# helenypzhang/Subspace-Multimodal-Learning

Measured on AMD Instinct MI355X. Metric: bags/sec fwd+bwd, DeformCrossTransMIL N=10k x 512, higher is better.
Workload: dtype f32

## Files before the change

### include/smml.h

```cpp
#ifndef SMML_H_
#define SMML_H_

#include <stddef.h>

#define SMML_ABI_VERSION 2

#ifdef __cplusplus
extern "C" {
#endif

const char* smml_last_error(void);
int smml_abi_version(void);
int smml_device_check(int device);
void* smml_event_create(void);
int smml_event_destroy(void* ev);
int smml_event_record(void* ev, void* stream);
int smml_event_elapsed_ms(void* start, void* stop, float* ms);

int smml_gemm_f32(const float* A, const float* B, float* C, const float* bias, const float* residual,
                  int M, int N, int K, long long sam, long long sak, long long sbk, long long sbn,
                  long long ldc, long long ldr, int nb0, int nb1, long long sa0, long long sa1,
                  long long sb0, long long sb1, long long sc0, long long sc1, long long sbias0,
                  long long sbias1, int bias_mode, int rows_per_bias, long long bias_ld, int act,
                  int splitk, int accumulate, float alpha, float beta, void* stream);
size_t smml_gemm_f32_det_workspace_bytes(int M, int N, int nb0, int nb1, int splitk);
int smml_gemm_f32_det(const float* A, const float* B, float* C, const float* bias, const float* residual,
                      int M, int N, int K, long long sam, long long sak, long long sbk, long long sbn,
                      long long ldc, long long ldr, int nb0, int nb1, long long sa0, long long sa1,
                      long long sb0, long long sb1, long long sc0, long long sc1, long long sbias0,
                      long long sbias1, int bias_mode, int rows_per_bias, long long bias_ld, int act,
                      int splitk, int accumulate, float alpha, float beta, void* workspace, size_t workspace_bytes,
                      void* stream);
void smml_gemm_force_generic(int on);
void smml_gemm_set_mode(int mode);
int smml_gemm_get_mode(void);
void smml_gemm_set_small_tile(int v);

int smml_gemm_b16(const void* A, const void* B, void* C, const float* bias, int M, int N, int K, long long lda, long long ldb,
                  long long ldc, int trans, int out_bf16, int splitk, void* stream);
void smml_gemm_b16_set_tile(int mode);
void smml_gemm_b16_set_slice_major(int on);
int smml_gemm_b16_batched(const void* A, const void* B, void* C, const float* bias, int M, int N, int K, long long lda, long long ldb,
                          long long ldc, int trans, int out_bf16, int splitk, int nb, long long sa, long long sb, long long sc, void* stream);

int smml_grouped_pointwise_applies(int groups, int cin_g, int cout_g);
int smml_grouped_pointwise_fwd_f32(const float* x, const float* w, float* y, long long rows, int groups, int cin_g, int cout_g, void* stream);
int smml_grouped_pointwise_dx_f32(const float* dy, const float* w, float* dx, long long rows, int groups, int cin_g, int cout_g, void* stream);
size_t smml_grouped_pointwise_dw_workspace_bytes(long long rows, int groups, int cin_g, int cout_g);
int smml_grouped_pointwise_dw_f32(const float* dy, const float* x, float* dw, long long rows, int groups, int cin_g, int cout_g,
                                  void* workspace, size_t workspace_bytes, void* stream);

int smml_layernorm_fwd_f32(const float* x, const float* gamma, const float* beta, float* y, float* mean,
                           float* rstd, long long R, int C, float eps, void* stream);
int smml_layernorm_fwd_mean_f32(const float* x, const float* gamma, const float* beta, float* mean, float* rstd, float* out, int nb,
                                long long n, int C, float eps, void* stream);
size_t smml_layernorm_fwd_mean_det_workspace_bytes(int nb, long long n, int C);
int smml_layernorm_fwd_mean_det_f32(const float* x, const float* gamma, const float* beta, float* mean, float* rstd, float* out, int nb,
                                    long long n, int C, float eps, void* workspace, size_t workspace_bytes, void* stream);
int smml_layernorm_bwd_f32(const float* x, const float* dy, const float* gamma, const float* mean,
                           const float* rstd, float* dx, float* dgamma, float* dbeta, long long R, int C,
                           long long rows_per_dy, float dy_scale, int accumulate_dx, void* stream);
size_t smml_layernorm_bwd_det_workspace_bytes(long long R, int C);
int smml_layernorm_bwd_det_f32(const float* x, const float* dy, const float* gamma, const float* mean,
                               const float* rstd, float* dx, float* dgamma, float* dbeta, long long R, int C,
                               long long rows_per_dy, float dy_scale, int accumulate_dx, void* workspace,
                               size_t workspace_bytes, void* stream);

int smml_colsum_f32(const float* x, float* out, int nb, long long R, int C, float scale, void* stream);
size_t smml_colsum_det_workspace_bytes(int nb, long long R, int C);
int smml_colsum_det_f32(const float* x, float* out, int nb, long long R, int C, float scale, void* workspace,
                        size_t workspace_bytes, void* stream);

int smml_orth_loss_f32(const float* P, const float* Ph, const float* G, const float* Gh, const float* dloss, float* loss,
                       float* dP, float* dPh, float* dG, float* dGh, int B, int D, float gamma, void* stream);

int smml_batchloss_tail_f32(const float* go, const float* gv, const float* dloss, float* loss, float* dgo, float* dgv, int R, int nv,
                            float n_total, void* stream);

int smml_relu_bwd_f32(const float* dy, const float* y, float* dx, long long n, void* stream);

int smml_offsets_out_len(int s, int ks, int r);
int smml_offsets_fwd_f32(const float* q, const float* w0, const float* b0, const float* w2, float* vgrid,
                         float* vs, int B, int Hh, int Ww, int G, int dg, int ks, int r, int posdim,
                         float offset_scale, void* stream);
size_t smml_offsets_bwd_workspace_bytes(int B, int Hh, int Ww, int G, int dg, int ks, int r, int posdim);
int smml_offsets_bwd_f32(const float* q, const float* w0, const float* b0, const float* w2,
                         const float* dvgrid, const float* dvs, float* dq, float* dw0, float* db0,
                         float* dw2, void* workspace, size_t workspace_bytes, int B, int Hh, int Ww, int G, int dg,
                         int ks, int r, int posdim, float offset_scale, int accumulate_dq, void* stream);

int smml_bilinear_sample_fwd_f32(const float* x, const float* vs, float* kv, int B, int Hh, int Ww, int G,
                                 int cg, int J, int posdim, void* stream);
int smml_bilinear_sample_bwd_f32(const float* x, const float* vs, const float* dkv, float* dx, float* dvs,
                                 int B, int Hh, int Ww, int G, int cg, int J, int posdim, void* stream);
size_t smml_bilinear_sample_bwd_det_workspace_bytes(int B, int Hh, int Ww, int G, int J);
int smml_bilinear_sample_bwd_det_f32(const float* x, const float* vs, const float* dkv, float* dx, float* dvs,
                                     void* workspace, size_t workspace_bytes, int B, int Hh, int Ww, int G, int cg,
                                     int J, int posdim, void* stream);
int smml_bilinear_corners_f32(const float* vs, int* cx, int* cy, unsigned char* cm, int n, int Hh, int Ww,
                              int posdim, void* stream);

typedef struct SmmlDeformOpts {
  const unsigned long long* seed_offset;
  int raw_distance;
  const unsigned short* mask_table;
  float mask_table_pmax;
  unsigned short* export_masks;
  int region_lds_cap;
} SmmlDeformOpts;

int smml_deform_attn_nst(int N);
int smml_deform_attn_fwd_f32(const float* q, const float* k, const float* v, const float* vs, const float* gq,
                             const float* w1, const float* b1, const float* w2, const float* b2,
                             const float* w3, const float* b3, float* out, float* lse, float* logits_t,
                             unsigned short* relu_masks, int B, int N, int J, int H, int G, int posdim, float scale,
                             float dropout_p, unsigned long long dropout_seed, void* ev_start, void* ev_stop, void* stream, const SmmlDeformOpts* opts);
size_t smml_deform_attn_bwd_workspace_bytes(int B, int N, int J, int H);
int smml_deform_attn_bwd_f32(const float* q, const float* k, const float* v, const float* vs, const float* gq,
                             const float* w1, const float* b1, const float* w2, const float* b2,
// ... 242 lines not shown
```

### subspace-multimodal-learning_amd/_capi.py

```python
from __future__ import annotations

import ctypes as C
import os
import re
from typing import Optional

import torch

_PKG = os.path.dirname(os.path.abspath(__file__))
LIB_PATH = os.environ.get("SMML_LIB") or os.path.join(_PKG, "lib", "libsmml_hip.so")

HEADER_PATH = os.path.join(os.path.dirname(_PKG), "include", "smml.h")


class DeformOpts(C.Structure):
    """SmmlDeformOpts of include/smml.h: optional behaviour of ONE fused deformable-attention launch, passed with the call.
    _fields_ are the header's, set below."""


_SCALARS = {"int": C.c_int, "long long": C.c_longlong, "unsigned long long": C.c_ulonglong, "float": C.c_float, "size_t": C.c_size_t}


def _ctype(ctext: str, where: str, ret: bool = False):
    t = " ".join(ctext.replace("*", " * ").split())
    if t == "void" and ret:
        return None
    if t == "const char *" and ret:
        return C.c_char_p
    if t == "const SmmlDeformOpts *":
        return C.POINTER(DeformOpts)
    if re.fullmatch(r"(const )?\w+( \w+)* \*", t):
        return C.c_void_p
    if t not in _SCALARS:
        raise RuntimeError(f"include/smml.h: type `{ctext.strip()}` of `{where}` is not one the ctypes binding knows")
    return _SCALARS[t]


def _declarator(text: str, where: str):
    m = re.fullmatch(r"\s*([\w\s]*[\w*])\s*\b([A-Za-z_]\w*)\s*", text)
    if not m or m.group(2) in ("int", "long", "float", "void", "unsigned", "size_t", "char", "short", "const"):
        raise RuntimeError(f"include/smml.h: cannot read `{text.strip()}` of `{where}` as `type name`")
    return m.group(2), _ctype(m.group(1), where), re.sub(r"\bconst\b|\s", "", m.group(1)) == "float*"


def parse_prototypes(text: str, params: Optional[dict] = None) -> dict:
    text = re.sub(r"/\*.*?\*/|//[^\n]*", " ", text, flags=re.S)
    text = re.sub(r"^[ \t]*#.*$", " ", text, flags=re.M)
    text = re.sub(r'extern\s+"C"\s*\{(.*)\}', r"\1", text, flags=re.S)
    sigs = {}
    *protos, tail = text.split(";")
    if tail.strip():
        raise RuntimeError(f"include/smml.h: `{' '.join(tail.split())}` does not end in `;`")
    for proto in protos:
        m = re.fullmatch(r"\s*([\w\s*]+?)\b(smml_\w+)\s*\(([^()]*)\)\s*", proto)
        if not m or m.group(2) in sigs:
            raise RuntimeError(f"include/smml.h: cannot read `{' '.join(proto.split())}` as one prototype `ret smml_name(type name, ...)`")
        ret, name, plist = m.groups()
        decl = [] if plist.strip() == "void" else [_declarator(p, name) for p in plist.split(",")]
        sigs[name] = (_ctype(ret, name, ret=True), [t for _, t, _ in decl])
        if params is not None:
            params[name] = decl
    return sigs


def parse_header(text: str, params: Optional[dict] = None):
    text = re.sub(r"/\*.*?\*/|//[^\n]*", " ", text, flags=re.S)
    abi = re.search(r"^[ \t]*#[ \t]*define[ \t]+SMML_ABI_VERSION[ \t]+(\d+)[ \t]*$", text, re.M)
    struct = re.search(r"typedef\s+struct\s+SmmlDeformOpts\s*\{(.*?)\}\s*SmmlDeformOpts\s*;", text, re.S)
    if not abi or not struct:
        raise RuntimeError("include/smml.h: SMML_ABI_VERSION or struct SmmlDeformOpts not found")
    fields = [_declarator(f, "SmmlDeformOpts")[:2] for f in struct.group(1).split(";") if f.strip()]
    return int(abi.group(1)), fields, parse_prototypes(text[:struct.start()] + text[struct.end():], params)


if not os.path.exists(HEADER_PATH):
    raise RuntimeError(f"{HEADER_PATH} is missing: the ctypes binding is derived from it (it ships with the repository, next to the package)")
PARAMS: dict = {}
with open(HEADER_PATH) as _h:
    ABI_VERSION, DeformOpts._fields_, SIGNATURES = parse_header(_h.read(), PARAMS)

_lib: Optional[C.CDLL] = None


def lib() -> C.CDLL:
    global _lib
    if _lib is None:
        if not os.path.exists(LIB_PATH):
            raise RuntimeError(
                f"{LIB_PATH} is missing: build it with `python -c 'import __graft_entry__ as g; g.build()'` "
                "(hipcc --offload-arch=gfx950); there is no CPU or eager fallback for this path")
        handle = C.CDLL(LIB_PATH)
        for name, (res, args) in SIGNATURES.items():
            fn = getattr(handle, name)
            fn.restype = res
            fn.argtypes = args
        if handle.smml_abi_version() != ABI_VERSION:
            raise RuntimeError(f"{LIB_PATH} implements C-ABI version {handle.smml_abi_version()}, this package binds version {ABI_VERSION}: rebuild it")
        if os.environ.get("SMML_GEMM_MODE"):
            handle.smml_gemm_set_mode(int(os.environ["SMML_GEMM_MODE"]))
        if os.environ.get("SMML_GEMM_SMALL_TILE"):
            handle.smml_gemm_set_small_tile(int(os.environ["SMML_GEMM_SMALL_TILE"]))
        _lib = handle
    return _lib


def deform_opts(seed_offset: Optional[torch.Tensor] = None, log_distance: bool = True, mask_table: Optional[torch.Tensor] = None,
                mask_table_pmax: float = 0.0, export_masks: Optional[torch.Tensor] = None, region_lds_cap: int = 0):
    if seed_offset is None and log_distance and mask_table is None and export_masks is None and not region_lds_cap:
        return None
    if seed_offset is not None and (seed_offset.dtype != torch.int64 or seed_offset.numel() != 1):
        raise RuntimeError("dropout_seed_offset must be a device int64 tensor with one element")
    o = DeformOpts(ptr(seed_offset), 0 if log_distance else 1, ptr(mask_table), float(mask_table_pmax), ptr(export_masks), int(region_lds_cap))
    return C.byref(o)


def check(rc: int, what: str = "") -> None:
    if rc != 0:
        msg = lib().smml_last_error().decode("utf-8", "replace")
        raise RuntimeError(f"smml call failed ({rc}){': ' + what if what else ''}: {msg}")


def ptr(t: Optional[torch.Tensor]):
    if t is None:
        return None
    if not t.is_cuda:
        raise RuntimeError("smml kernels need tensors resident in GPU HBM (got a CPU tensor); "
                           "this path has no CPU fallback")
    if not t.is_contiguous():
        raise RuntimeError("smml kernels need contiguous tensors")
    if t.device.index != torch.cuda.current_device():
        raise RuntimeError(f"smml kernels launch on the current device (cuda:{torch.cuda.current_device()}) but got a tensor on "
                           f"{t.device}; call torch.cuda.set_device first (one process per GPU)")
    return C.c_void_p(t.data_ptr())


def fptr(t: Optional[torch.Tensor]):
    if t is not None and t.dtype != torch.float32:
        raise RuntimeError(f"smml fp32 kernel got dtype {t.dtype}")
    return ptr(t)


def stream(device=None):
    return C.c_void_p(torch.cuda.current_stream(device).cuda_stream)


def _plan(decl):
    return [(pname, fptr if is_float else ptr if ctype is C.c_void_p else None) for pname, ctype, is_float in decl]


_PLANS = {name: _plan(decl) for name, decl in PARAMS.items()}


def bind(name: str, values, params: Optional[dict] = None) -> list:
    out = []
    for pname, conv in _PLANS[name] if params is None else _plan(params[name]):
        try:
            v = values[pname]
        except KeyError:
            raise RuntimeError(f"{name}: no value for its parameter `{pname}`") from None
        out.append(conv(v) if conv is not None and isinstance(v, torch.Tensor) else v)
    return out


def call(name: str, values, keys=None):
    if keys is not None and values.keys() != keys:
        raise RuntimeError(f"{name}: the namespace holds {sorted(values)}, its key set names {sorted(keys)}")
    return getattr(lib(), name)(*bind(name, values))
```

### subspace-multimodal-learning_amd/csrc/gemm.hip

```cpp
#include "smml_common.h"
#include <atomic>

namespace {

constexpr int BM = 128, BN = 64, BK = 16;
constexpr int LDA = BM + 4, LDB = BN + 4;

struct GemmArgs {
  const float* A; const float* B; float* C; const float* bias; const float* residual;
  int M, N, K;
  long long sam, sak, sbk, sbn, ldc, ldr;
  int nb0, nb1;
  long long sa0, sa1, sb0, sb1, sc0, sc1, sbias0, sbias1;
  int bias_mode, rows_per_bias; long long bias_ld;
  int act, splitk; float alpha, beta;
  int atomic;
  int swap_xy;
  long long scs;
};

template <bool GATE>
__device__ __forceinline__ float apply_act(float v, int act, int n, int N) {
  if (act == 1) return fmaxf(v, 0.f);
  if (act == 2) return tanhf(v);
  if constexpr (GATE) {
    if (act == 3 || (act == 4 && 2 * n >= N)) return 1.f / (1.f + expf(-v));
    if (act == 4) return tanhf(v);
  }
  return v;
}

template <bool GATE>
__global__ __launch_bounds__(256) void gemm_f32_kernel(GemmArgs g) {
  __shared__ float As[BK][LDA];
  __shared__ float Bs[BK][LDB];
  const int tid = threadIdx.x, wave = tid >> 6, lane = tid & 63, c = lane & 31, hf = lane >> 5;
  const int zb = blockIdx.z / g.splitk, ks = blockIdx.z - zb * g.splitk;
  const int b0 = zb / g.nb1, b1 = zb - b0 * g.nb1;
  const float* A = g.A + b0 * g.sa0 + b1 * g.sa1;
  const float* B = g.B + b0 * g.sb0 + b1 * g.sb1;
  float* C = g.C + b0 * g.sc0 + b1 * g.sc1 + ks * g.scs;
  const int m0 = (g.swap_xy ? blockIdx.y : blockIdx.x) * BM, n0 = (g.swap_xy ? blockIdx.x : blockIdx.y) * BN;
  const int ktiles = (g.K + BK - 1) / BK;
  const int tps = (ktiles + g.splitk - 1) / g.splitk;
  const int kt0 = ks * tps, kt1 = min(ktiles, kt0 + tps);

  floatx16 acc0 = {0}, acc1 = {0};
  const bool a_kcontig = (g.sak == 1);
  const bool b_kcontig = (g.sbk == 1) && (g.sbn != 1);

  for (int kt = kt0; kt < kt1; ++kt) {
    const int k0 = kt * BK;
    __syncthreads();
    if (a_kcontig) {
      const int k = tid & 15;
#pragma unroll
      for (int i = 0; i < 8; ++i) {
        const int m = (tid >> 4) + 16 * i;
        const int gm = m0 + m, gk = k0 + k;
        As[k][m] = (gm < g.M && gk < g.K) ? A[gm * g.sam + gk] : 0.f;
      }
    } else {
      const int m = tid & 127;
#pragma unroll
      for (int i = 0; i < 8; ++i) {
        const int k = (tid >> 7) + 2 * i;
        const int gm = m0 + m, gk = k0 + k;
        As[k][m] = (gm < g.M && gk < g.K) ? A[gm * g.sam + gk * g.sak] : 0.f;
      }
    }
    if (b_kcontig) {
      const int k = tid & 15;
#pragma unroll
      for (int i = 0; i < 4; ++i) {
        const int n = (tid >> 4) + 16 * i;
        const int gn = n0 + n, gk = k0 + k;
        Bs[k][n] = (gn < g.N && gk < g.K) ? B[gk + gn * g.sbn] : 0.f;
      }
    } else {
      const int n = tid & 63;
#pragma unroll
      for (int i = 0; i < 4; ++i) {
        const int k = (tid >> 6) + 4 * i;
        const int gn = n0 + n, gk = k0 + k;
        Bs[k][n] = (gn < g.N && gk < g.K) ? B[gk * g.sbk + gn * g.sbn] : 0.f;
      }
    }
    __syncthreads();
#pragma unroll
    for (int st = 0; st < BK / 2; ++st) {
      const float a = As[2 * st + hf][wave * 32 + c];
      acc0 = mfma32(a, Bs[2 * st + hf][c], acc0);
      acc1 = mfma32(a, Bs[2 * st + hf][32 + c], acc1);
    }
  }

  const float* bias = g.bias ? g.bias + b0 * g.sbias0 + b1 * g.sbias1 : nullptr;
  const float* res = g.residual ? g.residual + b0 * g.sc0 + b1 * g.sc1 : nullptr;
#pragma unroll
  for (int t = 0; t < 2; ++t) {
    const int n = n0 + 32 * t + c;
// ... 122 lines not shown
    store_tile();
    __syncthreads();
    if (kt + 1 < kt1) load_tile(kt + 1);
    float af[MI][8], bf[NI][8];
#pragma unroll
    for (int mi = 0; mi < MI; ++mi) {
      const int row = wm * (FBM / 2) + mi * 32 + c;
      if (A_KC) {
        const float4 x = *reinterpret_cast<const float4*>(&As[row * A_LD + 8 * hf]);
        const float4 y = *reinterpret_cast<const float4*>(&As[row * A_LD + 8 * hf + 4]);
        af[mi][0] = x.x; af[mi][1] = x.y; af[mi][2] = x.z; af[mi][3] = x.w;
        af[mi][4] = y.x; af[mi][5] = y.y; af[mi][6] = y.z; af[mi][7] = y.w;
      } else {
#pragma unroll
        for (int st = 0; st < 8; ++st) af[mi][st] = As[(8 * hf + st) * A_LD + row];
      }
    }
#pragma unroll
    for (int ni = 0; ni < NI; ++ni) {
      const int col = wn * (BN_ / 2) + ni * 32 + c;
      if (B_KC) {
        const float4 x = *reinterpret_cast<const float4*>(&Bs[col * B_LD + 8 * hf]);
        const float4 y = *reinterpret_cast<const float4*>(&Bs[col * B_LD + 8 * hf + 4]);
        bf[ni][0] = x.x; bf[ni][1] = x.y; bf[ni][2] = x.z; bf[ni][3] = x.w;
        bf[ni][4] = y.x; bf[ni][5] = y.y; bf[ni][6] = y.z; bf[ni][7] = y.w;
      } else {
#pragma unroll
        for (int st = 0; st < 8; ++st) bf[ni][st] = Bs[(8 * hf + st) * B_LD + col];
      }
    }
#pragma unroll
    for (int st = 0; st < 8; ++st)
#pragma unroll
      for (int mi = 0; mi < MI; ++mi)
#pragma unroll
        for (int ni = 0; ni < NI; ++ni) acc[mi][ni] = mfma32(af[mi][st], bf[ni][st], acc[mi][ni]);
  }

  const float* bias = g.bias ? g.bias + b0 * g.sbias0 + b1 * g.sbias1 : nullptr;
  const float* res = g.residual ? g.residual + b0 * g.sc0 + b1 * g.sc1 : nullptr;
  if (!g.atomic && m0 + FBM <= g.M && n0 + BN_ <= g.N) {
#pragma unroll
    for (int mi = 0; mi < MI; ++mi)
#pragma unroll
      for (int ni = 0; ni < NI; ++ni) {
        const int n = n0 + wn * (BN_ / 2) + ni * 32 + c;
        const int mb = m0 + wm * (FBM / 2) + mi * 32;
        float rv[16];
#pragma unroll
        for (int r = 0; r < 16; ++r) rv[r] = res ? res[(long long)(mb + acc_row(r, hf)) * g.ldr + n] : 0.f;
#pragma unroll
        for (int r = 0; r < 16; ++r) {
          const int m = mb + acc_row(r, hf);
          float v = g.alpha * acc[mi][ni][r];
          if (bias) v += (g.bias_mode == 2) ? bias[(m / g.rows_per_bias) * g.bias_ld + n] : bias[n];
          v = apply_act<GATE>(v, g.act, n, g.N);
          C[(long long)m * g.ldc + n] = fmaf(g.beta, rv[r], v);
        }
      }
    return;
  }
#pragma unroll
  for (int mi = 0; mi < MI; ++mi)
#pragma unroll
    for (int ni = 0; ni < NI; ++ni) {
      const int n = n0 + wn * (BN_ / 2) + ni * 32 + c;
      if (n >= g.N) continue;
#pragma unroll
      for (int r = 0; r < 16; ++r) {
        const int m = m0 + wm * (FBM / 2) + mi * 32 + acc_row(r, hf);
        if (m >= g.M) continue;
        float v = g.alpha * acc[mi][ni][r];
        if (g.atomic) {
          if (bias && ks == 0) v += (g.bias_mode == 2) ? bias[(m / g.rows_per_bias) * g.bias_ld + n] : bias[n];
          atomicAdd(&C[m * g.ldc + n], v);
        } else {
          if (bias) v += (g.bias_mode == 2) ? bias[(m / g.rows_per_bias) * g.bias_ld + n] : bias[n];
          v = apply_act<GATE>(v, g.act, n, g.N);
          if (res) v = fmaf(g.beta, res[m * g.ldr + n], v);
          C[m * g.ldc + n] = v;
        }
      }
    }
}

__device__ __forceinline__ uint2v f16_pack4(const float4 v) {
  typedef _Float16 h2 __attribute__((ext_vector_type(2)));
  const float2v a = {v.x, v.y}, b = {v.z, v.w};
  return (uint2v){__builtin_bit_cast(unsigned, __builtin_convertvector(a, h2)), __builtin_bit_cast(unsigned, __builtin_convertvector(b, h2))};
}
__device__ __forceinline__ floatx16 mfma16h(bf16x8 a, bf16x8 b, floatx16 c) {
  typedef _Float16 h8 __attribute__((ext_vector_type(8)));
  return __builtin_amdgcn_mfma_f32_32x32x16_f16(__builtin_bit_cast(h8, a), __builtin_bit_cast(h8, b), c, 0, 0, 0);
}

template <int BN_, bool A_KC, bool B_KC, int TERMS = 3, int FBM = 128, bool F16 = false>
__global__ __launch_bounds__(256, 2) void gemm_bf3_kernel(GemmArgs g) {
  static_assert(!F16 || TERMS == 1, "the fp16 form is single-term");
  constexpr int FBK = 32, NI = BN_ / 64, MI = FBM / 64;
  constexpr int A_LD = A_KC ? (FBK + 8) : (FBM + 32);
  constexpr int B_LD = B_KC ? (FBK + 8) : (BN_ + 32);
  constexpr int A_PLANE = (A_KC ? FBM : FBK) * A_LD, B_PLANE = (B_KC ? BN_ : FBK) * B_LD;
  constexpr int NA = FBM / 32, NB = BN_ / 32, MQ = FBM / 4;
  __shared__ __attribute__((aligned(16))) __bf16 As[TERMS * A_PLANE];
  __shared__ __attribute__((aligned(16))) __bf16 Bs[TERMS * B_PLANE];
  const int tid = threadIdx.x, wave = tid >> 6, lane = tid & 63, c = lane & 31, hf = lane >> 5;
  const int wm = wave >> 1, wn = wave & 1;
  const int zb = blockIdx.z / g.splitk, ks = blockIdx.z - zb * g.splitk;
  const int b0 = zb / g.nb1, b1 = zb - b0 * g.nb1;
  const float* A = g.A + b0 * g.sa0 + b1 * g.sa1;
  const float* B = g.B + b0 * g.sb0 + b1 * g.sb1;
  float* C = g.C + b0 * g.sc0 + b1 * g.sc1 + ks * g.scs;
  const int m0 = (g.swap_xy ? blockIdx.y : blockIdx.x) * FBM, n0 = (g.swap_xy ? blockIdx.x : blockIdx.y) * BN_;
  const int ktiles = (g.K + FBK - 1) / FBK;
  const int tps = (ktiles + g.splitk - 1) / g.splitk;
  const int kt0 = ks * tps, kt1 = min(ktiles, kt0 + tps);

  float4 ra[NA], rb[NB];
  auto load_tile = [&](int kt) {
    const int k0 = kt * FBK;
#pragma unroll
    for (int i = 0; i < NA; ++i) {
      const int idx = tid + 256 * i;
      if (A_KC) {
        const int row = idx >> 3, kq = idx & 7;
        const long long gm = min(m0 + row, g.M - 1);
        ra[i] = (k0 + 4 * kq < g.K) ? *reinterpret_cast<const float4*>(A + gm * g.sam + k0 + 4 * kq) : make_float4(0.f, 0.f, 0.f, 0.f);
      } else {
        const int k = idx / MQ, mq = idx - k * MQ;
        const int gm = m0 + 4 * mq;
        const float* p = A + (long long)min(k0 + k, g.K - 1) * g.sak;
        if (k0 + k >= g.K) ra[i] = make_float4(0.f, 0.f, 0.f, 0.f);
        else if (gm >= g.M) ra[i] = make_float4(0.f, 0.f, 0.f, 0.f);
        else if (gm + 3 < g.M) ra[i] = *reinterpret_cast<const float4*>(p + gm);
        else ra[i] = make_float4(p[min(gm, g.M - 1)], p[min(gm + 1, g.M - 1)], p[min(gm + 2, g.M - 1)], p[min(gm + 3, g.M - 1)]);
      }
    }
#pragma unroll
    for (int i = 0; i < NB; ++i) {
      const int idx = tid + 256 * i;
      if (B_KC) {
        const int row = idx >> 3, kq = idx & 7;
        const long long gn = min(n0 + row, g.N - 1);
        rb[i] = (k0 + 4 * kq < g.K) ? *reinterpret_cast<const float4*>(B + gn * g.sbn + k0 + 4 * kq) : make_float4(0.f, 0.f, 0.f, 0.f);
      } else {
        constexpr int NQ = BN_ / 4;
        const int k = idx / NQ, nq = idx - k * NQ;
        const int gn = n0 + 4 * nq;
        const float* p = B + (long long)min(k0 + k, g.K - 1) * g.sbk;
        if (k0 + k >= g.K) rb[i] = make_float4(0.f, 0.f, 0.f, 0.f);
        else if (gn >= g.N) rb[i] = make_float4(0.f, 0.f, 0.f, 0.f);
        else if (gn + 3 < g.N) rb[i] = *reinterpret_cast<const float4*>(p + gn);
        else rb[i] = make_float4(p[min(gn, g.N - 1)], p[min(gn + 1, g.N - 1)], p[min(gn + 2, g.N - 1)], p[min(gn + 3, g.N - 1)]);
      }
    }
  };
  auto store_tile = [&]() {
#pragma unroll
    for (int i = 0; i < NA; ++i) {
      const int idx = tid + 256 * i;
      const int off = A_KC ? ((idx >> 3) * A_LD + 4 * (idx & 7)) : ((idx / MQ) * A_LD + 4 * (idx % MQ));
      uint2v h, m, l;
      if (F16) h = f16_pack4(ra[i]); else split4_bf3(ra[i], h, m, l);
      *reinterpret_cast<uint2v*>(&As[off]) = h;
      if (TERMS == 3) {
        *reinterpret_cast<uint2v*>(&As[A_PLANE + off]) = m;
// ... 74 lines not shown
        }
    }
  }

  const float* bias = g.bias ? g.bias + b0 * g.sbias0 + b1 * g.sbias1 : nullptr;
  const float* res = g.residual ? g.residual + b0 * g.sc0 + b1 * g.sc1 : nullptr;
  if (!g.atomic && m0 + FBM <= g.M && n0 + BN_ <= g.N) {
#pragma unroll
    for (int mi = 0; mi < MI; ++mi)
#pragma unroll
      for (int ni = 0; ni < NI; ++ni) {
        const int n = n0 + wn * (BN_ / 2) + ni * 32 + c;
        const int mb = m0 + wm * (FBM / 2) + mi * 32;
        float rv[16];
#pragma unroll
        for (int r = 0; r < 16; ++r) rv[r] = res ? res[(long long)(mb + acc_row(r, hf)) * g.ldr + n] : 0.f;
#pragma unroll
        for (int r = 0; r < 16; ++r) {
          const int m = mb + acc_row(r, hf);
          float v = g.alpha * acc[mi][ni][r];
          if (bias) v += (g.bias_mode == 2) ? bias[(m / g.rows_per_bias) * g.bias_ld + n] : bias[n];
          v = apply_act<false>(v, g.act, n, g.N);
          C[(long long)m * g.ldc + n] = fmaf(g.beta, rv[r], v);
        }
      }
    return;
  }
#pragma unroll
  for (int mi = 0; mi < MI; ++mi)
#pragma unroll
    for (int ni = 0; ni < NI; ++ni) {
      const int n = n0 + wn * (BN_ / 2) + ni * 32 + c;
      if (n >= g.N) continue;
#pragma unroll
      for (int r = 0; r < 16; ++r) {
        const int m = m0 + wm * (FBM / 2) + mi * 32 + acc_row(r, hf);
        if (m >= g.M) continue;
        float v = g.alpha * acc[mi][ni][r];
        if (g.atomic) {
          if (bias && ks == 0) v += (g.bias_mode == 2) ? bias[(m / g.rows_per_bias) * g.bias_ld + n] : bias[n];
          atomicAdd(&C[m * g.ldc + n], v);
        } else {
          if (bias) v += (g.bias_mode == 2) ? bias[(m / g.rows_per_bias) * g.bias_ld + n] : bias[n];
          v = apply_act<false>(v, g.act, n, g.N);
          if (res) v = fmaf(g.beta, res[m * g.ldr + n], v);
          C[m * g.ldc + n] = v;
        }
      }
    }
}

__global__ __launch_bounds__(256) void gemm_det_reduce_kernel(const float* __restrict__ part, float* __restrict__ C, int M, int N,
                                                              long long ldc, int nb0, int nb1, long long sc0, long long sc1, int splitk,
                                                              int fold0, int fold1, int accumulate) {
  const int e1 = fold1 ? 1 : nb1;
  const long long mn = (long long)M * N;
  const long long total = (long long)(fold0 ? 1 : nb0) * e1 * mn;
  const long long idx = (long long)blockIdx.x * blockDim.x + threadIdx.x;
  if (idx >= total) return;
  const long long o = idx / mn, r = idx - o * mn;
  const int o0 = (int)(o / e1), o1 = (int)(o - (long long)o0 * e1);
  const int b0a = fold0 ? 0 : o0, b0b = fold0 ? nb0 : o0 + 1;
  const int b1a = fold1 ? 0 : o1, b1b = fold1 ? nb1 : o1 + 1;
  float s = 0.f;
  for (int b0 = b0a; b0 < b0b; ++b0)
    for (int b1 = b1a; b1 < b1b; ++b1) {
      const float* p = part + ((long long)b0 * nb1 + b1) * splitk * mn + r;
      for (int ks = 0; ks < splitk; ++ks) s += p[ks * mn];
    }
  const long long m = r / N, n = r - m * N;
  float* c = C + o0 * sc0 + o1 * sc1 + m * ldc + n;
  *c = accumulate ? *c + s : s;
}

}

static std::atomic<int> g_force_generic{0};
static std::atomic<int> g_mode{0};
extern "C" void smml_gemm_force_generic(int on) { g_force_generic = on; }
extern "C" void smml_gemm_set_mode(int mode) { g_mode = mode; }
extern "C" int smml_gemm_get_mode(void) { return g_mode; }
static std::atomic<int> g_small_tile{0};
extern "C" void smml_gemm_set_small_tile(int v) { g_small_tile = v; }

static int gemm_f32_run(const char* fn, const float* A, const float* B, float* C, const float* bias, const float* residual,
                        int M, int N, int K, long long sam, long long sak, long long sbk, long long sbn,
                        long long ldc, long long ldr, int nb0, int nb1, long long sa0, long long sa1,
                        long long sb0, long long sb1, long long sc0, long long sc1, long long sbias0,
                        long long sbias1, int bias_mode, int rows_per_bias, long long bias_ld, int act,
                        int splitk, int atomic, long long scs, float alpha, float beta, void* stream) {
  SMML_REQUIRE(A && B && C, "%s: null operand", fn);
  SMML_REQUIRE(M > 0 && N > 0 && K > 0 && nb0 > 0 && nb1 > 0, "%s: non-positive size (M=%d N=%d K=%d)", fn, M, N, K);
  SMML_REQUIRE(splitk >= 1, "%s: splitk must be >= 1", fn);
  SMML_REQUIRE(!((atomic || scs) && (act != 0 || residual)), "%s: split-K / accumulate excludes activation/residual", fn);
  SMML_REQUIRE(bias_mode >= 0 && bias_mode <= 2, "%s: bad bias_mode %d", fn, bias_mode);
  SMML_REQUIRE(bias_mode != 2 || rows_per_bias > 0, "%s: rows_per_bias must be positive", fn);
  SMML_REQUIRE(act >= 0 && act <= 4, "%s: bad activation %d", fn, act);
  SMML_REQUIRE(act != 4 || N % 2 == 0, "%s: activation 4 (tanh | sigmoid halves) needs an even N, got %d", fn, N);
  const long long gz = (long long)nb0 * nb1 * splitk;
  const long long gy = (N + BN - 1) / BN, gx = (M + BM - 1) / BM;
  const int swap_xy = gy > 65535;
  SMML_REQUIRE(gz <= 65535 && (swap_xy ? gx : gy) <= 65535,
               "smml_gemm_f32: grid too large (batch*splitk=%lld, row tiles=%lld, col tiles=%lld)", gz, gx, gy);
  GemmArgs g{A, B, C, bias_mode ? bias : nullptr, residual, M, N, K, sam, sak, sbk, sbn, ldc, ldr, nb0, nb1,
             sa0, sa1, sb0, sb1, sc0, sc1, sbias0, sbias1, bias_mode, rows_per_bias > 0 ? rows_per_bias : 1,
             bias_ld, act, splitk, alpha, beta, atomic, swap_xy, scs};
  SMML_REQUIRE(!bias_mode || bias, "smml_gemm_f32: bias_mode set but bias is null");
  auto al4 = [](long long v) { return (v & 3) == 0; };
  auto al16 = [](const void* p) { return (((size_t)p) & 15) == 0; };
  const bool a_kc = (sak == 1), a_mc = (sam == 1 && sak != 1);
  const bool b_kc = (sbk == 1 && sbn != 1), b_nc = (sbn == 1);
  const bool a_ok = al16(A) && al4(sa0) && al4(sa1) && ((a_kc && al4(sam)) || (a_mc && al4(sak)));
  const bool b_ok = al16(B) && al4(sb0) && al4(sb1) && ((b_kc && al4(sbn)) || (b_nc && al4(sbk)));
  const bool k_ok = (!a_kc && !b_kc) || (K % 4) == 0;
  const bool gate = act >= 3;
  if (a_ok && b_ok && k_ok && !g_force_generic) {
    const int bn = (N > 64 && gx * ((N + 127) / 128) * gz >= 1024) ? 128 : 64;
    const long long fy = (N + bn - 1) / bn;
    const bool small = bn == 64 && M > 64 && (g_small_tile == 2 || (g_small_tile == 0 && gx * fy * gz < 512));
    const long long fx = small ? (M + 63) / 64 : gx;
    const int fswap = fy > 65535;
    SMML_REQUIRE((fswap ? fx : fy) <= 65535, "smml_gemm_f32: grid too large");
    g.swap_xy = fswap;
    dim3 grid((unsigned)(fswap ? fy : fx), (unsigned)(fswap ? fx : fy), (unsigned)gz);
    hipStream_t st = (hipStream_t)stream;
    const bool bf3_mode = (g_mode == 2) || (g_mode == 0 && K >= 2048 && M >= 1024 && N >= 1024);
    const bool bf3 = !gate && bf3_mode;
    const bool bf1 = !gate && (g_mode == 3), f1 = !gate && (g_mode == 4);
#define SMML_FAST(BNV, AK, BK2)                                                                   \
  do {                                                                                            \
    if (f1) hipLaunchKernelGGL((gemm_bf3_kernel<BNV, AK, BK2, 1, 128, true>), grid, dim3(256), 0, st, g); \
    else if (bf1) hipLaunchKernelGGL((gemm_bf3_kernel<BNV, AK, BK2, 1>), grid, dim3(256), 0, st, g);   \
    else if (bf3) hipLaunchKernelGGL((gemm_bf3_kernel<BNV, AK, BK2>), grid, dim3(256), 0, st, g); \
    else if (gate) hipLaunchKernelGGL((gemm_f32_fast_kernel<BNV, AK, BK2, 128, true>), grid, dim3(256), 0, st, g); \
    else hipLaunchKernelGGL((gemm_f32_fast_kernel<BNV, AK, BK2>), grid, dim3(256), 0, st, g);     \
  } while (0)
#define SMML_SMALL(AK, BK2)                                                                          \
  do {                                                                                               \
    if (f1) hipLaunchKernelGGL((gemm_bf3_kernel<64, AK, BK2, 1, 64, true>), grid, dim3(256), 0, st, g);   \
    else if (bf1) hipLaunchKernelGGL((gemm_bf3_kernel<64, AK, BK2, 1, 64>), grid, dim3(256), 0, st, g);   \
    else if (bf3) hipLaunchKernelGGL((gemm_bf3_kernel<64, AK, BK2, 3, 64>), grid, dim3(256), 0, st, g); \
    else if (gate) hipLaunchKernelGGL((gemm_f32_fast_kernel<64, AK, BK2, 64, true>), grid, dim3(256), 0, st, g); \
    else hipLaunchKernelGGL((gemm_f32_fast_kernel<64, AK, BK2, 64>), grid, dim3(256), 0, st, g);     \
  } while (0)
    if (small) {
      if (a_kc && b_kc) SMML_SMALL(true, true); else if (a_kc) SMML_SMALL(true, false);
      else if (b_kc) SMML_SMALL(false, true); else SMML_SMALL(false, false);
    } else if (bn == 128) {
      if (a_kc && b_kc) SMML_FAST(128, true, true); else if (a_kc) SMML_FAST(128, true, false);
      else if (b_kc) SMML_FAST(128, false, true); else SMML_FAST(128, false, false);
    } else {
      if (a_kc && b_kc) SMML_FAST(64, true, true); else if (a_kc) SMML_FAST(64, true, false);
      else if (b_kc) SMML_FAST(64, false, true); else SMML_FAST(64, false, false);
    }
#undef SMML_FAST
#undef SMML_SMALL
    SMML_LAUNCH_CHECK("smml_gemm_f32/fast");
    return SMML_OK;
  }
  dim3 grid((unsigned)(swap_xy ? gy : gx), (unsigned)(swap_xy ? gx : gy), (unsigned)gz);
  if (gate) hipLaunchKernelGGL(gemm_f32_kernel<true>, grid, dim3(256), 0, (hipStream_t)stream, g);
  else hipLaunchKernelGGL(gemm_f32_kernel<false>, grid, dim3(256), 0, (hipStream_t)stream, g);
  SMML_LAUNCH_CHECK("smml_gemm_f32");
  return SMML_OK;
}

extern "C" int smml_gemm_f32(const float* A, const float* B, float* C, const float* bias, const float* residual,
                             int M, int N, int K, long long sam, long long sak, long long sbk, long long sbn,
                             long long ldc, long long ldr, int nb0, int nb1, long long sa0, long long sa1,
                             long long sb0, long long sb1, long long sc0, long long sc1, long long sbias0,
                             long long sbias1, int bias_mode, int rows_per_bias, long long bias_ld, int act,
                             int splitk, int accumulate, float alpha, float beta, void* stream) {
  const int atomic = (splitk > 1 || accumulate) ? 1 : 0;
  return gemm_f32_run("smml_gemm_f32", A, B, C, bias, residual, M, N, K, sam, sak, sbk, sbn, ldc, ldr, nb0, nb1, sa0, sa1, sb0, sb1,
                      sc0, sc1, sbias0, sbias1, bias_mode, rows_per_bias, bias_ld, act, splitk, atomic, 0, alpha, beta, stream);
}

extern "C" size_t smml_gemm_f32_det_workspace_bytes(int M, int N, int nb0, int nb1, int splitk) {
  if (M <= 0 || N <= 0 || nb0 <= 0 || nb1 <= 0 || splitk <= 0) return 0;
  return (size_t)nb0 * (size_t)nb1 * (size_t)splitk * (size_t)M * (size_t)N * sizeof(float);
}

extern "C" int smml_gemm_f32_det(const float* A, const float* B, float* C, const float* bias, const float* residual,
                                 int M, int N, int K, long long sam, long long sak, long long sbk, long long sbn,
                                 long long ldc, long long ldr, int nb0, int nb1, long long sa0, long long sa1,
                                 long long sb0, long long sb1, long long sc0, long long sc1, long long sbias0,
                                 long long sbias1, int bias_mode, int rows_per_bias, long long bias_ld, int act,
                                 int splitk, int accumulate, float alpha, float beta, void* workspace, size_t workspace_bytes,
                                 void* stream) {
  SMML_REQUIRE(A && B && C && workspace, "smml_gemm_f32_det: null operand or workspace");
  SMML_REQUIRE(M > 0 && N > 0 && K > 0 && nb0 > 0 && nb1 > 0 && splitk >= 1, "smml_gemm_f32_det: non-positive size (M=%d N=%d K=%d)", M, N, K);
  SMML_REQUIRE(!bias && !residual && bias_mode == 0 && act == 0, "smml_gemm_f32_det: the reduced product takes no bias, activation or residual");
  SMML_REQUIRE((long long)nb0 * nb1 * splitk <= 65535, "smml_gemm_f32_det: batch * splitk = %lld exceeds 65535", (long long)nb0 * nb1 * splitk);
  SMML_REQUIRE(workspace_bytes >= smml_gemm_f32_det_workspace_bytes(M, N, nb0, nb1, splitk), "smml_gemm_f32_det: workspace too small");
  const long long mn = (long long)M * N;
  float* part = (float*)workspace;
  int rc = gemm_f32_run("smml_gemm_f32_det", A, B, part, nullptr, nullptr, M, N, K, sam, sak, sbk, sbn, N, 0, nb0, nb1, sa0, sa1, sb0, sb1,
                        (long long)nb1 * splitk * mn, (long long)splitk * mn, 0, 0, 0, 1, 0, 0, splitk, 0, mn, alpha, 1.f, stream);
  if (rc) return rc;
  const int fold0 = (nb0 > 1 && sc0 == 0), fold1 = (nb1 > 1 && sc1 == 0);
  const long long total = (long long)(fold0 ? 1 : nb0) * (fold1 ? 1 : nb1) * mn;
  SMML_REQUIRE((total + 255) / 256 <= 2147483647LL, "smml_gemm_f32_det: output too large");
  hipLaunchKernelGGL(gemm_det_reduce_kernel, dim3((unsigned)((total + 255) / 256)), dim3(256), 0, (hipStream_t)stream, part, C, M, N, ldc,
                     nb0, nb1, sc0, sc1, splitk, fold0, fold1, accumulate ? 1 : 0);
  SMML_LAUNCH_CHECK("smml_gemm_f32_det/reduce");
  return SMML_OK;
}
```

Before: 1271.

## Add tall-skinny f32 GEMM kernel with wave-quantization-aware row tiling

Adds a dedicated MFMA-based f32 GEMM kernel for tall matrices with small N*K. It uses 128-column tiles and a variable row-tile height chosen by a planner that minimises wave-quantization cost over the device's slot count. The default-mode planner routes qualifying non-batched, non-split GEMMs (such as the N=10k instance projections) to it. This adds another code path with register-prefetch single buffering and different epilogue residual ordering, which could be slower for some shapes.

```diff
diff --git a/include/smml.h b/include/smml.h
--- a/include/smml.h
+++ b/include/smml.h
@@ -35,6 +35,9 @@
 void smml_gemm_set_mode(int mode);
 int smml_gemm_get_mode(void);
 void smml_gemm_set_small_tile(int v);
+void smml_gemm_set_tall(int v);
+int smml_gemm_tall_plan(const void* A, const void* B, int M, int N, int K, long long sam, long long sak, long long sbk, long long sbn,
+                        int nb0, int nb1, int act, int splitk, int partial, int mode, int slots, int* workgroups);
 
 int smml_gemm_b16(const void* A, const void* B, void* C, const float* bias, int M, int N, int K, long long lda, long long ldb,
                   long long ldc, int trans, int out_bf16, int splitk, void* stream);
diff --git a/subspace-multimodal-learning_amd/_capi.py b/subspace-multimodal-learning_amd/_capi.py
--- a/subspace-multimodal-learning_amd/_capi.py
+++ b/subspace-multimodal-learning_amd/_capi.py
@@ -100,6 +100,8 @@
             handle.smml_gemm_set_mode(int(os.environ["SMML_GEMM_MODE"]))
         if os.environ.get("SMML_GEMM_SMALL_TILE"):
             handle.smml_gemm_set_small_tile(int(os.environ["SMML_GEMM_SMALL_TILE"]))
+        if os.environ.get("SMML_GEMM_TALL"):
+            handle.smml_gemm_set_tall(int(os.environ["SMML_GEMM_TALL"]))
         _lib = handle
     return _lib
 
diff --git a/subspace-multimodal-learning_amd/csrc/gemm.hip b/subspace-multimodal-learning_amd/csrc/gemm.hip
--- a/subspace-multimodal-learning_amd/csrc/gemm.hip
+++ b/subspace-multimodal-learning_amd/csrc/gemm.hip
@@ -17,6 +17,7 @@
   int atomic;
   int swap_xy;
   long long scs;
+  int ofbm;
 };
 
 template <bool GATE>
@@ -305,6 +306,124 @@
         }
       }
     }
+}
+
+template <int MI, bool B_KC, int KS>
+__global__ __launch_bounds__(256, 2) void gemm_f32_tall_kernel(GemmArgs g) {
+  constexpr int FBK = 16, SK = FBK * KS, TM = 32 * MI, TN = 128;
+  constexpr int QPR = SK / 4, RS = 256 / QPR;
+  constexpr int A_LD = SK + 4, B_LD = B_KC ? (SK + 4) : (TN + 4);
+  constexpr int NA = (TM * QPR + 255) / 256, NB = TN * QPR / 256;
+  __shared__ __attribute__((aligned(16))) float As[TM * A_LD];
+  __shared__ __attribute__((aligned(16))) float Bs[(B_KC ? TN : SK) * B_LD];
+  const int tid = threadIdx.x, wave = tid >> 6, lane = tid & 63, c = lane & 31, hf = lane >> 5;
+  const float* A = g.A;
+  const float* B = g.B;
+  float* C = g.C;
+  const int m0 = blockIdx.x * TM, n0 = blockIdx.y * TN;
+  const int kstages = (g.K + SK - 1) / SK;
+
+  float4 ra[NA], rb[NB];
+  const int r0 = tid / QPR, q4 = 4 * (tid % QPR);
+  auto a_live = [&](int i) { return TM * QPR % 256 == 0 || i + 1 < NA || r0 + RS * i < TM; };
+  auto load_tile = [&](int ks) {
+    const int k0 = ks * SK;
+#pragma unroll
+    for (int i = 0; i < NA; ++i)
+      if (a_live(i)) {
+        const float* p = A + (long long)min(m0 + r0 + RS * i, g.M - 1) * g.sam + q4;
+        ra[i] = (k0 + q4 < g.K) ? *reinterpret_cast<const float4*>(p + k0) : make_float4(0.f, 0.f, 0.f, 0.f);
+      }
+#pragma unroll
+    for (int i = 0; i < NB; ++i) {
+      if (B_KC) {
+        const float* p = B + (long long)(n0 + r0 + RS * i) * g.sbn + q4;
+        rb[i] = (k0 + q4 < g.K) ? *reinterpret_cast<const float4*>(p + k0) : make_float4(0.f, 0.f, 0.f, 0.f);
+      } else {
+        const int idx = tid + 256 * i, k = k0 + (idx >> 5);
+        rb[i] = (k < g.K) ? *reinterpret_cast<const float4*>(B + (long long)k * g.sbk + n0 + 4 * (idx & 31)) : make_float4(0.f, 0.f, 0.f, 0.f);
+      }
+    }
+  };
+  auto store_tile = [&]() {
+#pragma unroll
+    for (int i = 0; i < NA; ++i)
+      if (a_live(i)) *reinterpret_cast<float4*>(&As[(r0 + RS * i) * A_LD + q4]) = ra[i];
+#pragma unroll
+    for (int i = 0; i < NB; ++i) {
+      if (B_KC) *reinterpret_cast<float4*>(&Bs[(r0 + RS * i) * B_LD + q4]) = rb[i];
+      else { const int idx = tid + 256 * i; *reinterpret_cast<float4*>(&Bs[(idx >> 5) * B_LD + 4 * (idx & 31)]) = rb[i]; }
+    }
+  };
+
+  floatx16 acc[MI];
+#pragma unroll
+  for (int mi = 0; mi < MI; ++mi) acc[mi] = floatx16{0};
+
+  load_tile(0);
+  for (int ks = 0; ks < kstages; ++ks) {
+    __syncthreads();
+    store_tile();
+    __syncthreads();
+    if (ks + 1 < kstages) load_tile(ks + 1);
+    const int col = wave * 32 + c;
+#pragma unroll
+    for (int sub = 0; sub < KS; ++sub) {
+      if (sub > 0 && ks * SK + sub * FBK >= g.K) break;
+      float bf[8];
+      if (B_KC) {
+        const float4 x = *reinterpret_cast<const float4*>(&Bs[col * B_LD + sub * FBK + 8 * hf]);
+        const float4 y = *reinterpret_cast<const float4*>(&Bs[col * B_LD + sub * FBK + 8 * hf + 4]);
+        bf[0] = x.x; bf[1] = x.y; bf[2] = x.z; bf[3] = x.w;
+        bf[4] = y.x; bf[5] = y.y; bf[6] = y.z; bf[7] = y.w;
+      } else {
+#pragma unroll
+        for (int st = 0; st < 8; ++st) bf[st] = Bs[(sub * FBK + 8 * hf + st) * B_LD + col];
+      }
+#pragma unroll
+      for (int mi = 0; mi < MI; ++mi) {
+        const int row = mi * 32 + c;
+        const float4 x = *reinterpret_cast<const float4*>(&As[row * A_LD + sub * FBK + 8 * hf]);
+        const float4 y = *reinterpret_cast<const float4*>(&As[row * A_LD + sub * FBK + 8 * hf + 4]);
+        const float af[8] = {x.x, x.y, x.z, x.w, y.x, y.y, y.z, y.w};
+#pragma unroll
+        for (int st = 0; st < 8; ++st) acc[mi] = mfma32(af[st], bf[st], acc[mi]);
+      }
+    }
+  }
+
+  const float* bias = g.bias;
+  const float* res = g.residual;
+  const int n = n0 + wave * 32 + c;
+#pragma unroll
+  for (int mi = 0; mi < MI; ++mi) {
+    const int mb = m0 + mi * 32;
+    if (mb >= g.M) break;
+    if ((mb / g.ofbm + 1) * g.ofbm <= g.M) {
+      float rv[16];
+#pragma unroll
+      for (int r = 0; r < 16; ++r) rv[r] = res ? res[(long long)(mb + acc_row(r, hf)) * g.ldr + n] : 0.f;
+#pragma unroll
+      for (int r = 0; r < 16; ++r) {
+        const int m = mb + acc_row(r, hf);
+        float v = g.alpha * acc[mi][r];
+        if (bias) v += (g.bias_mode == 2) ? bias[(m / g.rows_per_bias) * g.bias_ld + n] : bias[n];
+        v = apply_act<false>(v, g.act, n, g.N);
+        C[(long long)m * g.ldc + n] = fmaf(g.beta, rv[r], v);
+      }
+    } else {
+#pragma unroll
+      for (int r = 0; r < 16; ++r) {
+        const int m = mb + acc_row(r, hf);
+        if (m >= g.M) continue;
+        float v = g.alpha * acc[mi][r];
+        if (bias) v += (g.bias_mode == 2) ? bias[(m / g.rows_per_bias) * g.bias_ld + n] : bias[n];
+        v = apply_act<false>(v, g.act, n, g.N);
+        if (res) v = fmaf(g.beta, res[(long long)m * g.ldr + n], v);
+        C[(long long)m * g.ldc + n] = v;
+      }
+    }
+  }
 }
 
 __device__ __forceinline__ uint2v f16_pack4(const float4 v) {
@@ -545,6 +664,48 @@
 extern "C" int smml_gemm_get_mode(void) { return g_mode; }
 static std::atomic<int> g_small_tile{0};
 extern "C" void smml_gemm_set_small_tile(int v) { g_small_tile = v; }
+static std::atomic<int> g_tall{0};
+extern "C" void smml_gemm_set_tall(int v) { g_tall = v; }
+
+static int gemm_tall_slots() {
+  static const int slots = [] {
+    int dev = 0, n = 0;
+    if (hipGetDevice(&dev) != hipSuccess || hipDeviceGetAttribute(&n, hipDeviceAttributeMultiprocessorCount, dev) != hipSuccess || n <= 0) {
+      (void)hipGetLastError();
+      n = 256;
+    }
+    return 2 * n;
+  }();
+  return slots;
+}
+
+extern "C" int smml_gemm_tall_plan(const void* A, const void* B, int M, int N, int K, long long sam, long long sak, long long sbk,
+                                   long long sbn, int nb0, int nb1, int act, int splitk, int partial, int mode, int slots,
+                                   int* workgroups) {
+  SMML_REQUIRE(workgroups, "smml_gemm_tall_plan: workgroups is null");
+  *workgroups = 0;
+  if (mode < 0 || mode == 1 || mode > 5) return 0;
+  if (M <= 0 || N <= 0 || K <= 0 || nb0 != 1 || nb1 != 1 || splitk != 1 || partial || act < 0 || act >= 3) return 0;
+  if (N % 128 != 0 || N / 128 > 65535 || K % 4 != 0 || sak != 1) return 0;
+  const bool b_kc = (sbk == 1 && sbn != 1), b_nc = (sbn == 1);
+  if ((((size_t)A) & 15) || (((size_t)B) & 15) || (sam & 3) || !((b_kc && !(sbn & 3)) || (b_nc && !(sbk & 3)))) return 0;
+  const long long ncol = N / 128;
+  int mi = mode;
+  if (mode == 0) {
+    if (slots <= 0) slots = gemm_tall_slots();
+    if ((((long long)M + 63) / 64) * ncol < 2LL * slots) return 0;
+    if ((long long)N * K < 96LL * ((long long)N + K) || (long long)N * K > 65536) return 0;
+    long long best = 0;
+    for (int t = 2; t <= 5; ++t) {
+      const long long wg = (((long long)M + 32 * t - 1) / (32 * t)) * ncol, cost = ((wg + slots - 1) / slots) * t;
+      if (mi == 0 || cost < best) { mi = t; best = cost; }
+    }
+  }
+  const long long wg = (((long long)M + 32 * mi - 1) / (32 * mi)) * ncol;
+  if (wg > 2147483647LL) return 0;
+  *workgroups = (int)wg;
+  return mi;
+}
 
 static int gemm_f32_run(const char* fn, const float* A, const float* B, float* C, const float* bias, const float* residual,
                         int M, int N, int K, long long sam, long long sak, long long sbk, long long sbn,
@@ -590,6 +751,27 @@
     const bool bf3_mode = (g_mode == 2) || (g_mode == 0 && K >= 2048 && M >= 1024 && N >= 1024);
     const bool bf3 = !gate && bf3_mode;
     const bool bf1 = !gate && (g_mode == 3), f1 = !gate && (g_mode == 4);
+    int tall_wg = 0;
+    const int tall = (bf3 || bf1 || f1) ? 0 : smml_gemm_tall_plan(A, B, M, N, K, sam, sak, sbk, sbn, nb0, nb1, act, splitk, atomic || scs, g_tall, 0, &tall_wg);
+    const int tall_ks = K >= 512 ? 2 : 1;
+    if (tall) {
+      g.ofbm = small ? 64 : 128;
+      const dim3 tgrid((unsigned)((M + 32 * tall - 1) / (32 * tall)), (unsigned)(N / 128), 1);
+#define SMML_TALL(MIV)                                                                                 \
+  do {                                                                                                 \
+    if (tall_ks == 2) {                                                                                \
+      if (b_kc) hipLaunchKernelGGL((gemm_f32_tall_kernel<MIV, true, 2>), tgrid, dim3(256), 0, st, g);  \
+      else hipLaunchKernelGGL((gemm_f32_tall_kernel<MIV, false, 2>), tgrid, dim3(256), 0, st, g);      \
+    } else {                                                                                           \
+      if (b_kc) hipLaunchKernelGGL((gemm_f32_tall_kernel<MIV, true, 1>), tgrid, dim3(256), 0, st, g);  \
+      else hipLaunchKernelGGL((gemm_f32_tall_kernel<MIV, false, 1>), tgrid, dim3(256), 0, st, g);      \
+    }                                                                                                  \
+  } while (0)
+      if (tall == 2) SMML_TALL(2); else if (tall == 3) SMML_TALL(3); else if (tall == 4) SMML_TALL(4); else SMML_TALL(5);
+#undef SMML_TALL
+      SMML_LAUNCH_CHECK("smml_gemm_f32/tall");
+      return SMML_OK;
+    }
 #define SMML_FAST(BNV, AK, BK2)                                                                   \
   do {                                                                                            \
     if (f1) hipLaunchKernelGGL((gemm_bf3_kernel<BNV, AK, BK2, 1, 128, true>), grid, dim3(256), 0, st, g); \
```

New measurement: 1280 (median of 3 runs). No clear change (+0.7%).
